# julien-michot/tinyopt

Measured on AMD Instinct MI355X. Metric: LM iterations/s (batched dense n<=50), higher is better.
Workload: dtype f32

## Files before the change

### include/tinyopt_amd.h

```cpp
#ifndef TINYOPT_AMD_H_
#define TINYOPT_AMD_H_

#include <stddef.h>
#include <stdint.h>

#ifdef __cplusplus
extern "C" {
#endif

#define TOA_VERSION 1

#define TOA_OK 0
#define TOA_E_ARG (-1)
#define TOA_E_HIP (-2)
#define TOA_E_NOMEM (-3)
#define TOA_E_UNSUPPORTED (-4)
#define TOA_E_RCCL (-5)

#define TOA_F32 0
#define TOA_F64 1

#define TOA_MODEL_DENSE_ROW 1
#define TOA_MODEL_GAUSSIAN_PRIOR 2
#define TOA_MODEL_SQRT2 3
// ... 206 lines not shown
#define TOA_DIFF_NUM_CENTRAL 2
#define TOA_DIFF_NUM_FAST_CENTRAL 3
typedef struct toa_jit_spec {
  int32_t dtype, num_params, residuals_per_item, scalars_per_item, header_scalars;
  int32_t manifold;
  int32_t kind;
  int32_t x_scalars;
  const char* plus_body;
  int32_t diff;
  float diff_h;
  union {
    int32_t reserved[4];
    int32_t large_n;
    struct {
      int32_t toa_pad0_;
      int32_t shared_scalars;
    };
  };
} toa_jit_spec;
int toa_model_compile_ex(toa_handle h, const toa_jit_spec* spec, const char* body, toa_jit_model* out, char* log_out, size_t log_cap);
int toa_jit_set_cache_dir(const char* dir);
int toa_jit_model_info(toa_jit_model m, int* from_cache, int* xdim);
int toa_jit_model_stats(toa_jit_model m, int* wg_per_cu, int* lds_bytes_per_wg, int* num_regs, int* scratch_bytes);
int toa_model_destroy(toa_jit_model m);
int toa_jit_lm_run(toa_handle h, toa_jit_model model, int num_items, int64_t P, const void* data_dev, void* x_dev,
                   const toa_options* options, const toa_results* results, uint64_t* counters_dev);
int toa_jit_accumulate(toa_handle h, toa_jit_model model, int num_items, int64_t P, const void* data_dev, const void* x_dev,
                       int want_grad, void* g_dev, void* H_dev, double* cost_dev, int32_t* nres_dev);
int toa_jit_check_gradient(toa_handle h, toa_jit_model model, int num_items, int64_t P, const void* data_dev, const void* x_dev,
                           double eps, int method, int check_H, double* max_dist_dev, int32_t* ok_dev);
int toa_jit_eval(toa_handle h, toa_jit_model model, int num_items, int64_t P, const void* data_dev, const void* x_dev, void* res_dev,
                 void* J_dev);
typedef struct toa_gd_options {
  float lr;
  int32_t reserved[7];
} toa_gd_options;
void toa_gd_options_default(toa_gd_options* o);
int toa_jit_gd_run(toa_handle h, toa_jit_model model, int num_items, int64_t P, const void* data_dev, void* x_dev,
                   const toa_options* options, const toa_gd_options* gd, const toa_results* results, uint64_t* counters_dev);
int toa_jit_lm_run_split(toa_handle h, toa_jit_model model, int num_items, int64_t P, const void* data_dev, void* x_dev,
                         const toa_options* options, const toa_results* results, uint64_t* counters_dev, int splits);
int toa_jit_lm_begin(toa_handle h, toa_jit_model model, int num_items, int64_t P, const void* data_dev, void* x_dev,
                     const toa_options* options, const toa_results* results, void* state_dev);
int toa_jit_lm_step(toa_handle h, toa_jit_model model, int num_items, int64_t P, const void* data_dev, void* x_dev,
                    const toa_options* options, const toa_results* results, uint64_t* counters_dev, void* state_dev,
                    int32_t* active_dev);
// ... 77 lines not shown
```

### include/tinyopt_amd/tinyopt.hpp

```cpp
#pragma once

#include <array>
#include <chrono>
#include <cstdint>
#include <functional>
#include <iostream>
#include <limits>
#include <stdexcept>
#include <string>
#include <algorithm>
#include <type_traits>
#include <utility>
#include <vector>

#include "../tinyopt_amd.h"

namespace tinyopt_amd {

enum StopReason : int {
  kOutOfMemory = -4, kSolverFailed = -3, kSystemHasNaNOrInf = -2, kSkipped = -1, kNone = 0, kMinError, kMinRelError,
  kMinDeltaNorm, kMinGradNorm, kMaxIters, kMaxNoDecr, kMaxConsecNoDecr, kTimedOut, kUserStopped
};

struct Options {
// ... 348 lines not shown
    if (kind_ == TOA_JIT_COST_GGN_MULTI) detail::refuse_cost_ggn_multi("no ragged batches (bind_ragged)");
    if (kS_ > 0) detail::refuse_shared("no ragged batches (bind_ragged)");
    return RaggedJitModel<Scalar>(*this, counts, data, header);
  }
  const std::string& compile_log() const { return log_; }
  toa_jit_model handle() const { return h_; }
  const Context& ctx() const { return *ctx_; }
  int n() const { return n_; }
  int residuals_per_item() const { return kR_; }
  int item_scalars() const { return kD_; }
  int header_scalars() const { return kH_; }
  int xdim() const { return xdim_; }
  int diff() const { return diff_; }
  int manifold() const { return manifold_; }
  int kind() const { return kind_; }
  bool large_n() const { return large_n_; }
  int shared_scalars() const { return kS_; }
  struct PriorBuildStats { int wg_per_cu = 0, num_regs = 0, scratch_bytes = 0; };
  PriorBuildStats stats_prior(bool ragged = false) const {
    PriorBuildStats s;
    check(toa_jit_model_stats_prior(ctx_->get(), h_, ragged ? 1 : 0, &s.wg_per_cu, &s.num_regs, &s.scratch_bytes));
    return s;
  }
  struct BuildStats { int wg_per_cu = 0, lds_bytes_per_wg = 0, num_regs = 0, scratch_bytes = 0; };
  BuildStats stats() const {
    BuildStats s;
    check(toa_jit_model_stats(h_, &s.wg_per_cu, &s.lds_bytes_per_wg, &s.num_regs, &s.scratch_bytes));
    return s;
  }

 private:
  const Context* ctx_;
  toa_jit_model h_ = nullptr;
  int n_, kR_, kD_, kH_, xdim_, diff_, manifold_, kind_;
  bool large_n_;
  int kS_;
  std::string log_;
};
template <typename Scalar>
class PriorTag {
 public:
  bool has_prior() const { return prior_rows_ >= 0; }
  toa_prior prior_pod() const {
    toa_prior p{};
    p.mu_dev = prior_mu_.data(); p.W_dev = prior_W_.data(); p.rows = prior_rows_;
    return p;
  }

 protected:
  void set_prior(const JitResidual<Scalar>& res, int64_t P, const Scalar* mu, const Scalar* W, int rows) {
// ... 892 lines not shown
```

### tinyopt_amd/_capi.py

```python
from __future__ import annotations

import ctypes as C
import os

_HERE = os.path.dirname(os.path.abspath(__file__))
LIB_PATH = os.environ.get("TINYOPT_AMD_LIB", os.path.join(_HERE, "libtinyopt_amd.so"))

F32, F64 = 0, 1
MODEL_DENSE_ROW, MODEL_GAUSSIAN_PRIOR, MODEL_SQRT2, MODEL_SE3_REPROJ, MODEL_CIRCLE_FIT, MODEL_DENSE_ROW_AD6 = 1, 2, 3, 4, 5, 6
MODEL_TESTFN = 7
MODEL_MAHA_PRIOR = 8
MODEL_SE3_PRIOR = 9
MODEL_DENSE_ROW_NATURAL = 10
MODEL_DENSE_ROW_AD = 11

STOP_NAMES = {
    -4: "kOutOfMemory", -3: "kSolverFailed", -2: "kSystemHasNaNOrInf", -1: "kSkipped", 0: "kNone",
    1: "kMinError", 2: "kMinRelError", 3: "kMinDeltaNorm", 4: "kMinGradNorm", 5: "kMaxIters",
    6: "kMaxNoDecr", 7: "kMaxConsecNoDecr", 8: "kTimedOut", 9: "kUserStopped",
}


class ToaOptions(C.Structure):
    _fields_ = [
# ... 107 lines not shown
    "toa_dense_row_synth": (C.c_int, [_P, C.c_int, C.c_int, C.c_int, C.c_int64, C.c_uint64, C.c_int64, _P, _P, _P]),
    "toa_accumulate": (C.c_int, [_P, C.c_int, C.c_int, C.c_int, C.c_int, C.c_int64, _P, _P, C.c_int, _P, _P, _P, _P]),
    "toa_solve_damped": (C.c_int, [_P, C.c_int, C.c_int, C.c_int64, _P, _P, C.c_double, _P, _P]),
    "toa_inv_cov": (C.c_int, [_P, C.c_int, C.c_int, C.c_int64, _P, _P, _P]),
    "toa_lm_run": (C.c_int, [_P, C.c_int, C.c_int, C.c_int, C.c_int, C.c_int64, _P, _P, C.POINTER(ToaOptions),
                             C.POINTER(ToaResults), _P]),
    "toa_ba_lists_run": (C.c_int, [_P, C.c_int, C.c_int, C.c_int, C.c_int, C.c_int64, _P, _P, _P, _P, _P, C.POINTER(ToaOptions),
                                   C.POINTER(ToaResults), _P, C.c_double]),
    "toa_ba_run_constant": (C.c_int, [_P, C.c_int, C.c_int, C.c_int, C.c_int64, _P, _P, C.POINTER(ToaOptions), C.POINTER(ToaResults), _P,
                                      C.POINTER(ToaBaConstant)]),
    "toa_ba_lists_run_constant": (C.c_int, [_P, C.c_int, C.c_int, C.c_int, C.c_int, C.c_int64, _P, _P, _P, _P, _P, C.POINTER(ToaOptions),
                                            C.POINTER(ToaResults), _P, C.c_double, C.POINTER(ToaBaConstant)]),
    "toa_model_compile": (C.c_int, [_P, C.c_int, C.c_int, C.c_int, C.c_int, C.c_int, C.c_char_p, C.POINTER(_P), C.c_char_p, C.c_size_t]),
    "toa_abi_version": (C.c_int, []),
    "toa_device_count": (C.c_int, [C.POINTER(C.c_int)]),
    "toa_set_tuning": (C.c_int, [_P, C.POINTER(ToaTuning)]),
    "toa_get_tuning": (C.c_int, [_P, C.POINTER(ToaTuning)]),
    "toa_debug_timeline": (C.c_int, [_P, C.c_char_p]),
    "toa_model_compile_ex": (C.c_int, [_P, C.POINTER(ToaJitSpec), C.c_char_p, C.POINTER(_P), C.c_char_p, C.c_size_t]),
    "toa_jit_set_cache_dir": (C.c_int, [C.c_char_p]),
    "toa_lm_step_log": (C.c_int, [_P, C.c_int, C.c_int, C.c_int64, _P, _P, _P, _P]),
    "toa_jit_model_info": (C.c_int, [_P, C.POINTER(C.c_int), C.POINTER(C.c_int)]),
    "toa_jit_model_stats": (C.c_int, [_P, C.POINTER(C.c_int), C.POINTER(C.c_int), C.POINTER(C.c_int), C.POINTER(C.c_int)]),
    "toa_model_destroy": (C.c_int, [_P]),
    "toa_jit_lm_run": (C.c_int, [_P, _P, C.c_int, C.c_int64, _P, _P, C.POINTER(ToaOptions), C.POINTER(ToaResults), _P]),
    "toa_jit_accumulate": (C.c_int, [_P, _P, C.c_int, C.c_int64, _P, _P, C.c_int, _P, _P, _P, _P]),
    "toa_jit_check_gradient": (C.c_int, [_P, _P, C.c_int, C.c_int64, _P, _P, C.c_double, C.c_int, C.c_int, _P, _P]),
    "toa_jit_eval": (C.c_int, [_P, _P, C.c_int, C.c_int64, _P, _P, _P, _P]),
    "toa_jit_lm_run_ragged": (C.c_int, [_P, _P, _P, _P, C.c_int, C.c_int64, C.c_int64, _P, _P, C.POINTER(ToaOptions), C.POINTER(ToaResults), _P,
                                        C.c_uint32]),
    "toa_jit_gd_run_ragged": (C.c_int, [_P, _P, _P, _P, C.c_int, C.c_int64, C.c_int64, _P, _P, C.POINTER(ToaOptions), C.POINTER(ToaGdOptions),
                                        C.POINTER(ToaResults), _P, C.c_uint32]),
    "toa_jit_accumulate_ragged": (C.c_int, [_P, _P, _P, _P, C.c_int, C.c_int64, C.c_int64, _P, _P, C.c_int, _P, _P, _P, _P]),
    "toa_jit_eval_ragged": (C.c_int, [_P, _P, _P, _P, C.c_int, C.c_int64, C.c_int64, _P, _P, _P, _P]),
    "toa_jit_model_stats_ragged": (C.c_int, [_P, _P, C.POINTER(C.c_int), C.POINTER(C.c_int), C.POINTER(C.c_int)]),
    "toa_jit_lm_run_prior": (C.c_int, [_P, _P, C.c_int, C.c_int64, _P, _P, C.POINTER(ToaPrior), C.POINTER(ToaOptions), C.POINTER(ToaResults), _P]),
    "toa_jit_accumulate_prior": (C.c_int, [_P, _P, C.c_int, C.c_int64, _P, _P, C.POINTER(ToaPrior), C.c_int, _P, _P, _P, _P]),
    "toa_jit_lm_run_ragged_prior": (C.c_int, [_P, _P, _P, _P, C.c_int, C.c_int64, C.c_int64, _P, _P, C.POINTER(ToaPrior), C.POINTER(ToaOptions),
                                              C.POINTER(ToaResults), _P, C.c_uint32]),
    "toa_jit_accumulate_ragged_prior": (C.c_int, [_P, _P, _P, _P, C.c_int, C.c_int64, C.c_int64, _P, _P, C.POINTER(ToaPrior), C.c_int, _P, _P, _P, _P]),
    "toa_jit_model_stats_prior": (C.c_int, [_P, _P, C.c_int, C.POINTER(C.c_int), C.POINTER(C.c_int), C.POINTER(C.c_int)]),
    "toa_jit_lm_run_bounds": (C.c_int, [_P, _P, C.c_int, C.c_int64, _P, _P, C.POINTER(ToaBounds), C.POINTER(ToaPrior), C.POINTER(ToaOptions),
                                        C.POINTER(ToaResults), _P]),
    "toa_jit_lm_run_ragged_bounds": (C.c_int, [_P, _P, _P, _P, C.c_int, C.c_int64, C.c_int64, _P, _P, C.POINTER(ToaBounds), C.POINTER(ToaPrior),
                                               C.POINTER(ToaOptions), C.POINTER(ToaResults), _P, C.c_uint32]),
    "toa_jit_accumulate_bounds": (C.c_int, [_P, _P, C.c_int, C.c_int64, _P, _P, C.POINTER(ToaBounds), C.POINTER(ToaPrior), C.c_int, _P, _P, _P, _P]),
# ... 54 lines not shown
```

### tinyopt_amd/api.py

```python
from __future__ import annotations

import contextlib
import copy
import ctypes as C
import enum
import functools
import time

import numpy as np
from dataclasses import dataclass, field
from typing import Optional

import torch

from . import _capi
from ._capi import (F32, F64, MODEL_DENSE_ROW_AD, MODEL_DENSE_ROW_NATURAL, MODEL_TESTFN, MODEL_MAHA_PRIOR, MODEL_SE3_PRIOR, MODEL_CIRCLE_FIT, MODEL_DENSE_ROW, MODEL_DENSE_ROW_AD6, MODEL_GAUSSIAN_PRIOR, MODEL_SE3_REPROJ,
                    MODEL_SQRT2, ToaBaConstant, ToaBounds, ToaGdOptions, ToaJitSpec, ToaLbfgsOptions, ToaOptions, ToaPrior, ToaResults, ToaShared, check)


class StopReason(enum.IntEnum):
    kOutOfMemory = -4
    kSolverFailed = -3
    kSystemHasNaNOrInf = -2
    kSkipped = -1
# ... 797 lines not shown
        self._h = C.c_void_p()
        log = C.create_string_buffer(1 << 16)
        spec = ToaJitSpec()
        spec.dtype, spec.num_params, spec.residuals_per_item = _dtype_code(dtype), self.n, self.kR
        spec.scalars_per_item, spec.header_scalars = self.kD, self.kH
        spec.manifold, spec.kind = self.MANIFOLDS[manifold], self.KINDS[kind]
        spec.diff, spec.diff_h = self.DIFFS[diff], self.diff_h
        spec.large_n = 1 if self.large_n else 0
        spec.shared_scalars = self.kS
        if manifold == "user":
            if not plus_body or int(x_scalars) < 1:
                raise ValueError('manifold="user" needs plus_body (the body of x (+) d) and x_scalars')
            spec.x_scalars, spec.plus_body = int(x_scalars), plus_body.encode()
        rc = self.ctx.lib.toa_model_compile_ex(self.ctx.h, C.byref(spec), body.encode(), C.byref(self._h), log, len(log))
        self.compile_log = log.value.decode(errors="replace")
        check(rc)
        fc = C.c_int(0)
        check(self.ctx.lib.toa_jit_model_info(self._h, C.byref(fc), None))
        self.from_cache = bool(fc.value)

    def stats(self) -> dict:
        v = [C.c_int(0) for _ in range(4)]
        check(self.ctx.lib.toa_jit_model_stats(self._h, *[C.byref(t) for t in v]))
        return dict(wg_per_cu=v[0].value, lds_bytes_per_wg=v[1].value, num_regs=v[2].value, scratch_bytes=v[3].value)

    @staticmethod
    def set_cache_dir(path: Optional[str], ctx: Optional["Context"] = None) -> None:
        check((ctx or default_context()).lib.toa_jit_set_cache_dir(None if path is None else path.encode()))

    def bind(self, data: Optional[torch.Tensor], header: Optional[torch.Tensor] = None, items: int = 1,
             shared: Optional[torch.Tensor] = None) -> "JitModel":
        kS = getattr(self, "kS", 0)
        if shared is None:
            if kS:
                raise ValueError(f"bind: a model with shared_scalars = {kS} needs shared=, the batch's [items, {kS}] table")
            return JitModel(self, data, header, items)
        if not kS:
            raise ValueError("bind: shared= is the table of a model with shared_scalars > 0; this model has none")
        m = JitModel(self, data, header, items)
        if not isinstance(shared, torch.Tensor) or tuple(shared.shape) != (m.items, kS):
            raise ValueError(f"bind: shared must be an [items, shared_scalars] = [{m.items}, {kS}] tensor, not "
                             f"{list(shared.shape) if isinstance(shared, torch.Tensor) else type(shared).__name__}")
        if shared.dtype != self.dtype or shared.device != m.packed.device:
            raise ValueError(f"bind: shared must have the model's dtype {self.dtype} on the data's device {m.packed.device}, not {shared.dtype} on {shared.device}")
        m.shared = shared.contiguous()
        return m

# ... 728 lines not shown
```

### tinyopt_amd/csrc/jet.hpp

```cpp
#pragma once
#include <hip/hip_runtime.h>

#include <cmath>

namespace toa {

using ::sqrt; using ::sin; using ::cos; using ::tan; using ::atan; using ::atan2; using ::tanh;
using ::exp; using ::log; using ::pow; using ::fabs; using std::abs;
using ::isnan; using ::isinf; using ::isfinite; using ::signbit;
using ::acos; using ::asin; using ::sinh; using ::cosh; using ::cbrt; using ::exp2; using ::log2; using ::log10;
using ::log1p; using ::expm1; using ::hypot; using ::erf; using ::erfc; using ::floor; using ::ceil; using ::fmax;
using ::fmin; using ::fdim; using ::fma; using ::copysign;

template <typename T, int N>
struct Jet {
  T a;
  T v[N];

  __host__ __device__ Jet() : a(T(0)) {
#pragma unroll
    for (int i = 0; i < N; ++i) v[i] = T(0);
  }
  __host__ __device__ Jet(T value) : a(value) {
#pragma unroll
    for (int i = 0; i < N; ++i) v[i] = T(0);
  }
  __host__ __device__ Jet(T value, int k) : a(value) {
#pragma unroll
    for (int i = 0; i < N; ++i) v[i] = (i == k) ? T(1) : T(0);
  }
  __host__ __device__ Jet& operator+=(const Jet& y) { *this = *this + y; return *this; }
  __host__ __device__ Jet& operator-=(const Jet& y) { *this = *this - y; return *this; }
  __host__ __device__ Jet& operator*=(const Jet& y) { *this = *this * y; return *this; }
  __host__ __device__ Jet& operator/=(const Jet& y) { *this = *this / y; return *this; }
  __host__ __device__ Jet& operator+=(T s) { a += s; return *this; }
  __host__ __device__ Jet& operator-=(T s) { a -= s; return *this; }
  __host__ __device__ Jet& operator*=(T s) { *this = *this * s; return *this; }
  __host__ __device__ Jet& operator/=(T s) { *this = *this / s; return *this; }
};

#define TOA_JET_FN template <typename T, int N> __host__ __device__ inline
#define TOA_JET_LOOP _Pragma("unroll") for (int i = 0; i < N; ++i)

TOA_JET_FN Jet<T, N> operator+(const Jet<T, N>& f) { return f; }
TOA_JET_FN Jet<T, N> operator-(const Jet<T, N>& f) { Jet<T, N> r; r.a = -f.a; TOA_JET_LOOP r.v[i] = -f.v[i]; return r; }
TOA_JET_FN Jet<T, N> operator+(const Jet<T, N>& f, const Jet<T, N>& g) {
  Jet<T, N> r; r.a = f.a + g.a; TOA_JET_LOOP r.v[i] = f.v[i] + g.v[i]; return r;
}
TOA_JET_FN Jet<T, N> operator+(const Jet<T, N>& f, T s) { Jet<T, N> r = f; r.a += s; return r; }
TOA_JET_FN Jet<T, N> operator+(T s, const Jet<T, N>& f) { Jet<T, N> r = f; r.a += s; return r; }
TOA_JET_FN Jet<T, N> operator-(const Jet<T, N>& f, const Jet<T, N>& g) {
  Jet<T, N> r; r.a = f.a - g.a; TOA_JET_LOOP r.v[i] = f.v[i] - g.v[i]; return r;
}
TOA_JET_FN Jet<T, N> operator-(const Jet<T, N>& f, T s) { Jet<T, N> r = f; r.a -= s; return r; }
TOA_JET_FN Jet<T, N> operator-(T s, const Jet<T, N>& f) { Jet<T, N> r = -f; r.a += s; return r; }
TOA_JET_FN Jet<T, N> operator*(const Jet<T, N>& f, const Jet<T, N>& g) {
  Jet<T, N> r; r.a = f.a * g.a; TOA_JET_LOOP r.v[i] = f.a * g.v[i] + f.v[i] * g.a; return r;
}
TOA_JET_FN Jet<T, N> operator*(const Jet<T, N>& f, T s) { Jet<T, N> r; r.a = f.a * s; TOA_JET_LOOP r.v[i] = f.v[i] * s; return r; }
TOA_JET_FN Jet<T, N> operator*(T s, const Jet<T, N>& f) { return f * s; }
TOA_JET_FN Jet<T, N> operator/(const Jet<T, N>& f, const Jet<T, N>& g) {
// ... 162 lines not shown
TOA_JET_FN bool isnan(const Jet<T, N>& f) { return f.a != f.a; }
TOA_JET_FN bool isnormal(const Jet<T, N>& f) {
  const T m = f.a < T(0) ? -f.a : f.a;
  return ::isfinite(f.a) && m >= (sizeof(T) == 4 ? T(1.17549435e-38f) : T(2.2250738585072014e-308));
}
TOA_JET_FN bool signbit(const Jet<T, N>& f) { return ::signbit(f.a); }
TOA_JET_FN int fpclassify(const Jet<T, N>& f) {
  if (f.a != f.a) return 0;
  if (::isinf(f.a)) return 1;
  if (f.a == T(0)) return 2;
  return isnormal(f) ? 4 : 3;
}
TOA_JET_FN bool isless(const Jet<T, N>& f, const Jet<T, N>& g) { return f.a < g.a; }
TOA_JET_FN bool isgreater(const Jet<T, N>& f, const Jet<T, N>& g) { return f.a > g.a; }
TOA_JET_FN bool islessequal(const Jet<T, N>& f, const Jet<T, N>& g) { return f.a <= g.a; }
TOA_JET_FN bool isgreaterequal(const Jet<T, N>& f, const Jet<T, N>& g) { return f.a >= g.a; }
TOA_JET_FN bool islessgreater(const Jet<T, N>& f, const Jet<T, N>& g) { return f.a < g.a || f.a > g.a; }
TOA_JET_FN bool isunordered(const Jet<T, N>& f, const Jet<T, N>& g) { return f.a != f.a || g.a != g.a; }
TOA_JET_FN bool IsFinite(const Jet<T, N>& f) { return isfinite(f); }
TOA_JET_FN bool IsNaN(const Jet<T, N>& f) { return isnan(f); }
TOA_JET_FN bool IsNormal(const Jet<T, N>& f) { return isnormal(f); }
TOA_JET_FN bool IsInfinite(const Jet<T, N>& f) { return isinf(f); }

#undef TOA_JET_FN
#undef TOA_JET_LOOP

}
```

### tinyopt_amd/csrc/jit.hip

```cpp
#include <dlfcn.h>
#include <glob.h>
#include <sys/stat.h>
#include <unistd.h>

#include <cstdint>
#include <mutex>
#include <string>
#include <vector>

#include "kernels.hpp"
#include "gd_kernels.hpp"
#include "lbfgs_kernels.hpp"
#include "large_model_geom.hpp"
#include "_obj/jit_embed.inc"

struct JitObject {
  hipModule_t module = nullptr;
  hipFunction_t fn[5] = {};
  bool from_cache = false;
  int wg_per_cu = 0;
  int regs = 0, scratch = 0;
};
enum { kFnFused = 0, kFnSeam = 1 };
enum { kFnWideInit = 0, kFnWidePart, kFnWideStep, kFnWideStop, kFnWidePers };
// ... 7 lines not shown
  std::string prefix;
};
struct JitEvalGeom {
  size_t lds_j = 0, lds = 0;
  int items_j = 0, items = 0;
};
struct toa_jit_model_s {
  bool large_n = false;
  toa::LargeModelRows mr = {};
  enum { kObjWide = 2 * kForms, kObjEval = kObjWide + 1, kObjLarge = kObjEval + 2, kObjLbfgs = kObjLarge + 1, kObjects = kObjLbfgs + 2 };
  JitObject obj[kObjects];
  JitObject& form(int form, int robust) { return obj[2 * form + robust]; }
  JitObject& wide() { return obj[kObjWide]; }
  JitObject& eval(bool ragged) { return obj[kObjEval + (ragged ? 1 : 0)]; }
  JitObject& large() { return obj[kObjLarge]; }
  JitObject& lbfgs(bool ragged) { return obj[kObjLbfgs + (ragged ? 1 : 0)]; }
  JitGeom geom[2];
  JitEvalGeom ev_geom[2];
  int lbfgs_wg[2][17] = {};
  std::mutex build_mu;
  int dtype = 0, kN = 0, kR = 0, kD = 0, kH = 0, device = 0;
  int manifold = 0, kind = 0, xdim = 0, x_scalars = 0;
  int kS = 0;
  bool row_model = false;
  size_t memo_bytes = 0;
  hipStream_t last_stream = nullptr;
  std::vector<hipStream_t> streams;
  void used_on(hipStream_t s) {
    last_stream = s;
    for (hipStream_t t : streams) if (t == s) return;
    streams.push_back(s);
  }
  std::string functor_src, model_expr, arch;
  std::string wide_model_expr;
  bool wide_row_model = false;
  int diff = 0;
  double diff_h = 0;
  toa_jit_spec spec = {};
  std::string body;
  int body_kind = 0;
  bool seam_only = false;
  struct Twin { int method; double h; toa_jit_model_s* m; };
  std::vector<Twin> twins;
};

namespace {
// ... 270 lines not shown
  return ((dtype == TOA_F32 ? toa::WaveLds<float>::bytes(n) : toa::WaveLds<double>::bytes(n)) + 15) & ~size_t(15);
}

struct RowGeom { size_t stage_bytes, lds_wave, lds_wg; int carve_off; };
static RowGeom row_stage_geometry(toa_jit_model m, int waves_override) {
  const int n = m->kN, sz = m->dtype == TOA_F32 ? 4 : 8;
  const bool ad = m->kind != TOA_JIT_ACCUMULATE;
  int table = 0;
  if (ad && m->manifold == TOA_MANIFOLD_SE3) table = (12 * 7 * sz + 15) & ~15;
  if (ad && m->manifold == TOA_MANIFOLD_USER) {
    const int cwmax = jit_flag_int("TOA_AD_CW", 12);
    const int chunks = (n + cwmax - 1) / cwmax, cw = (n + chunks - 1) / chunks;
    table = (chunks * m->x_scalars * (cw + 1) * sz + 15) & ~15;
  }
  const int waves = waves_override ? waves_override : jit_flag_int("TOA_ROW_WAVES", TOA_ROW_WAVES);
  RowGeom g;
  g.stage_bytes = size_t(toa::RowStageGeom::make(sz, n, m->kR, m->kD, ad || jit_flag_int("TOA_ROW_SINGLE", TOA_ROW_SINGLE),
                                                 jit_flag_int("TOA_ROW_NBUF", TOA_ROW_NBUF), waves, table, m->kS).bytes);
  const size_t dead = std::min(m->dtype == TOA_F32 ? toa::WaveLds<float>::pass_dead_bytes(n) : toa::WaveLds<double>::pass_dead_bytes(n), g.stage_bytes);
  g.carve_off = int(g.stage_bytes - dead);
  g.lds_wave = carve_bytes(m->dtype, n) + size_t(g.carve_off);
  g.lds_wg = 4 * g.lds_wave;
  return g;
}

static bool is_cost_model(toa_jit_model m) { return m->kind == TOA_JIT_COST || m->kind == TOA_JIT_COST_GRAD; }
static bool is_hess_model(toa_jit_model m) { return m->kind == TOA_JIT_COST_HESS; }
static int refuse_hess_model(const std::string& who, const std::string& what) {
  return toa_fail(TOA_E_UNSUPPORTED, who + ": a second-order scalar cost (TOA_JIT_COST_HESS) runs in the uniform one-launch form through toa_jit_lm_run "
                                           "(LM / GN), toa_jit_accumulate, toa_jit_check_gradient and toa_jit_model_stats only: " + what);
}
static bool is_ggn_model(toa_jit_model m) { return m->kind == TOA_JIT_COST_GGN; }
static int refuse_ggn_model(const std::string& who, const std::string& what) {
  return toa_fail(TOA_E_UNSUPPORTED, who + ": a rank-one second-order scalar cost (TOA_JIT_COST_GGN) runs in the uniform one-launch form through toa_jit_lm_run "
                                           "(LM / GN), toa_jit_accumulate, toa_jit_check_gradient and toa_jit_model_stats only: " + what);
}
static bool is_ggn_multi_model(toa_jit_model m) { return m->kind == TOA_JIT_COST_GGN_MULTI; }
static int refuse_ggn_multi_model(const std::string& who, const std::string& what) {
  return toa_fail(TOA_E_UNSUPPORTED, who + ": a multi-output second-order scalar cost (TOA_JIT_COST_GGN_MULTI) runs in the uniform one-launch form through "
                                           "toa_jit_lm_run (LM / GN), toa_jit_accumulate, their _prior and _shared forms, toa_jit_check_gradient and "
                                           "toa_jit_model_stats only: " + what);
}
static bool is_item_cost_model(toa_jit_model m) { return is_ggn_model(m) || is_ggn_multi_model(m); }

static bool is_shared_model(toa_jit_model m) { return m->kS > 0; }
static int refuse_shared_model(const std::string& who, const std::string& what) {
// ... 529 lines not shown
            ", 0, TOA_ROBUST_>";
  } else if (row_model) {
    const std::string f = std::string("toa::UserFunctor<") + tname + ">";
    const std::string mf = std::to_string(spec->manifold);
    model = std::string("toa::RowModel<") + tname + ", " + std::to_string(lay.nbm) + ", " + std::to_string(lay.thin) + ", " +
            (spec->kind == TOA_JIT_ACCUMULATE ? f : std::string("toa::AdRowFunctor<") + tname + ", " + f + ", " + mf + ">") + ", " + mf + ", TOA_ROBUST_>";
  } else {
    model = std::string("toa::JetModel<") + tname + ", toa::UserFunctor<" + tname + ">, " + std::to_string(spec->manifold) + ", TOA_ROBUST_>";
  }
  const std::string jet_model = std::string("toa::JetModel<") + tname + ", toa::UserFunctor<" + tname + ">, " + std::to_string(spec->manifold) + ">";
  toa_jit_model_s* m = new (std::nothrow) toa_jit_model_s;
  if (!m) return toa_fail(TOA_E_NOMEM, "out of host memory");
  m->dtype = dtype; m->kN = n; m->kR = kR; m->kD = kD; m->kH = kH;
  m->manifold = spec->manifold; m->kind = spec->kind; m->row_model = row_model;
  m->x_scalars = user_manifold ? spec->x_scalars : 0;
  m->xdim = spec->manifold == TOA_MANIFOLD_SE3 ? 12 : (user_manifold ? spec->x_scalars : n);
  m->device = h->device;
  m->functor_src = src; m->model_expr = model; m->arch = arch;
  m->wide_row_model = row_model && n > 12 && kS == 0;
  m->kS = kS;
  m->diff = diff; m->diff_h = numeric ? diff_h : 0.0;
  m->spec = *spec; m->spec.plus_body = nullptr;
  m->body = body; m->body_kind = body_kind; m->seam_only = seam_only;
  if (large) {
    m->large_n = true;
    m->row_model = false; m->wide_row_model = false;
    if (int rc = build_large_model(m, log_out, log_cap)) { delete m; return rc; }
    *out = m;
    return TOA_OK;
  }
  if (cost_kind) {
    if (int rc = build_cost_variant(m, log_out, log_cap)) { delete m; return rc; }
    *out = m;
    return TOA_OK;
  }
  if (hess_kind) {
    if (int rc = build_hess_variant(m, log_out, log_cap)) { delete m; return rc; }
    *out = m;
    return TOA_OK;
  }
  if (ggn_kind || ggn_multi_kind) {
    m->wide_row_model = false;
    if (int rc = build_ggn_variant(m, log_out, log_cap)) { delete m; return rc; }
    *out = m;
    return TOA_OK;
  }
  {
    std::string wm = model;
    wm.replace(wm.find("TOA_ROBUST_"), 11, "true");
    m->wide_model_expr = m->wide_row_model ? wm : jet_model;
  }
  if (int rc = build_variant(m, 0, log_out, log_cap)) { delete m; return rc; }
  *out = m;
  return TOA_OK;
}
extern "C" {

int toa_model_compile_ex(toa_handle h, const toa_jit_spec* spec, const char* body, toa_jit_model* out, char* log_out, size_t log_cap) {
  if (!spec) return toa_fail(TOA_E_ARG, "toa_model_compile: null argument");
  return compile_model(h, spec, body, spec->kind, double(spec->diff_h), false, out, log_out, log_cap);
}

int toa_model_compile(toa_handle h, int dtype, int num_params, int residuals_per_item, int scalars_per_item, int header_scalars,
                      const char* residual_body, toa_jit_model* out, char* log_out, size_t log_cap) {
  toa_jit_spec spec;
  std::memset(&spec, 0, sizeof(spec));
  spec.dtype = dtype; spec.num_params = num_params; spec.residuals_per_item = residuals_per_item;
  spec.scalars_per_item = scalars_per_item; spec.header_scalars = header_scalars;
  return toa_model_compile_ex(h, &spec, residual_body, out, log_out, log_cap);
}

int toa_jit_model_info(toa_jit_model m, int* from_cache, int* xdim) {
  if (!m) return toa_fail(TOA_E_ARG, "toa_jit_model_info: null model");
  if (from_cache) *from_cache = (m->large_n ? m->large() : m->form(0, 0)).from_cache ? 1 : 0;
  if (xdim) *xdim = m->xdim;
  return TOA_OK;
}

int toa_jit_model_stats(toa_jit_model m, int* wg_per_cu, int* lds_bytes_per_wg, int* num_regs, int* scratch_bytes) {
  if (!m) return toa_fail(TOA_E_ARG, "toa_jit_model_stats: null model");
  TOA_ON_DEVICE(m->device);
  if (m->large_n) {
    const hipFunction_t fn = m->mr.rows_j;
    int v = 0;
    if (wg_per_cu) { if (hipModuleOccupancyMaxActiveBlocksPerMultiprocessor(&v, fn, 256, m->mr.lds_j) != hipSuccess || v < 1) v = 1; *wg_per_cu = v; }
    if (lds_bytes_per_wg) *lds_bytes_per_wg = int(m->mr.lds_j);
    if (num_regs) { HIP_TRY(hipFuncGetAttribute(&v, HIP_FUNC_ATTRIBUTE_NUM_REGS, fn)); *num_regs = v; }
    if (scratch_bytes) { HIP_TRY(hipFuncGetAttribute(&v, HIP_FUNC_ATTRIBUTE_LOCAL_SIZE_BYTES, fn)); *scratch_bytes = v; }
    return TOA_OK;
  }
  const JitObject& V = m->form(0, 0);
  if (wg_per_cu) *wg_per_cu = V.wg_per_cu;
  if (lds_bytes_per_wg) *lds_bytes_per_wg = int(m->geom[0].lds_wg);
  int v = 0;
  if (num_regs) { HIP_TRY(hipFuncGetAttribute(&v, HIP_FUNC_ATTRIBUTE_NUM_REGS, V.fn[kFnFused])); *num_regs = v; }
  if (scratch_bytes) { HIP_TRY(hipFuncGetAttribute(&v, HIP_FUNC_ATTRIBUTE_LOCAL_SIZE_BYTES, V.fn[kFnFused])); *scratch_bytes = v; }
  return TOA_OK;
}

int toa_model_destroy(toa_jit_model m) {
  if (!m) return TOA_OK;
  TOA_ON_DEVICE(m->device);
  for (hipStream_t s : m->streams) {
    if (stream_is_capturing(s))
      return toa_fail(TOA_E_UNSUPPORTED, "toa_model_destroy: a stream this model was launched on is being captured; end the capture first "
                                         "(and keep the model for as long as a graph that recorded its kernels may be launched)");
    (void)hipGetLastError();
  }
  for (hipStream_t s : m->streams) {
    if (hipStreamSynchronize(s) != hipSuccess) (void)hipGetLastError();
  }
  for (const toa_jit_model_s::Twin& t : m->twins) (void)toa_model_destroy(t.m);
  for (JitObject& O : m->obj) if (O.module) (void)hipModuleUnload(O.module);
  delete m;
  return TOA_OK;
}

}

// ... 830 lines not shown
  size_t gbytes = 0;
  if (hipError_t e = hipModuleGetGlobal(&gp, &gbytes, mod, "toa_eval_geom"); e != hipSuccess || gbytes != sizeof(geom))
    return fail("the code object does not carry its LDS geometry", e);
  if (hipError_t e = hipMemcpyDtoH(geom, gp, sizeof(geom)); e != hipSuccess) return fail("reading the LDS geometry", e);
  if (geom[0] < 16 || geom[2] < 16 || geom[1] < 1 || geom[3] < 1 || size_t(geom[0]) * 4 > 160 * 1024 || size_t(geom[2]) * 4 > 160 * 1024)
    return fail("implausible LDS geometry", hipErrorInvalidValue);
  for (int k = 0; k < 2; ++k)
    if (size_t(geom[2 * k]) * 4 > 64 * 1024)
      if (hipError_t e = hipFuncSetAttribute(reinterpret_cast<const void*>(fn[k]), hipFuncAttributeMaxDynamicSharedMemorySize, geom[2 * k] * 4); e != hipSuccess)
        return fail("raising the dynamic LDS limit to " + std::to_string(geom[2 * k] * 4) + " bytes per workgroup", e);
  JitObject& E = m->eval(ragged);
  JitEvalGeom& G = m->ev_geom[ragged ? 1 : 0];
  E.fn[kFnRowsJ] = fn[0]; E.fn[kFnRows] = fn[1];
  G.lds_j = size_t(geom[0]); G.lds = size_t(geom[2]);
  G.items_j = geom[1]; G.items = geom[3];
  E.from_cache = cached;
  E.module = mod;
  return TOA_OK;
}
static int ensure_eval(toa_jit_model m, hipStream_t stream, const bool ragged) {
  return lazy_build(m, stream, [&] { return m->eval(ragged).module != nullptr; },
                    "run-time model: the Eval kernels of this model are compiled on their first use (toa_jit_eval), which cannot "
                    "happen while the stream is being captured; run the call once before hipStreamBeginCapture",
                    [&] { return build_eval(m, ragged); });
}

static int launch_eval(const char* who, toa_handle h, toa_jit_model model, int num_items, int64_t P, const void* data_dev, const void* x_dev, void* res_dev,
                       void* J_dev, const toa::RaggedArgs* rag) {
  if (int rc = ensure_eval(model, h->stream, rag != nullptr)) return rc;
  const JitEvalGeom& E = model->ev_geom[rag ? 1 : 0];
  model->used_on(h->stream);
  const bool want_j = J_dev != nullptr;
  const hipFunction_t fn = model->eval(rag != nullptr).fn[want_j ? kFnRowsJ : kFnRows];
  const size_t pw = want_j ? E.lds_j : E.lds;
  const long long it = want_j ? E.items_j : E.items;
  const long long nss = ((long long)num_items + it - 1) / it;
  const long long want_units = (long long)h->num_cus * 32 * 4;
  long long spu = nss;
  if ((long long)P < want_units) spu = std::max(1ll, std::min(nss, nss * (long long)P / want_units));
  const long long upp = (nss + spu - 1) / spu;
  const long long grid = std::max(1ll, std::min(((long long)P * upp + 3) / 4, (long long)h->num_cus * 16));
  const void* d = data_dev;
  const void* x = x_dev;
  long long Pll = P;
  int items = num_items, spui = int(spu);
  toa::RaggedArgs ra = rag ? *rag : toa::RaggedArgs();
  void* args[] = {&d, &x, &Pll, &items, &res_dev, &J_dev, &spui, &ra};
// ... 168 lines not shown
```

### tinyopt_amd/csrc/row_model.hpp

```cpp
#pragma once
#include "shared.hpp"
#include "row_stage_geom.hpp"
#ifndef TOA_ROW_SINGLE
#define TOA_ROW_SINGLE 1
#endif
#ifndef TOA_ROW_XREGS
#define TOA_ROW_XREGS 0
#endif
#ifndef TOA_ROW_ABL
#define TOA_ROW_ABL 0
#endif

namespace toa {

__device__ __forceinline__ float seed_one(bool b, float) {
  return __builtin_bit_cast(float, __builtin_amdgcn_readfirstlane(b ? 0x3f800000 : 0));
}
__device__ __forceinline__ double seed_one(bool b, double) {
  const unsigned hi = unsigned(__builtin_amdgcn_readfirstlane(b ? 0x3ff00000 : 0));
  return __builtin_bit_cast(double, (unsigned long long)hi << 32);
}
template <typename T, int CW>
struct ChunkSeededX {
  const T* xs;
  int c0;
  __device__ __forceinline__ Jet<T, CW> operator[](int j) const {
    Jet<T, CW> r;
    r.a = xs[j];
#pragma unroll
    for (int s = 0; s < CW; ++s) r.v[s] = seed_one(j == c0 + s, T(0));
    return r;
  }
};
template <typename T, int CW>
struct ChunkSeededD {
  int c0;
  __device__ __forceinline__ Jet<T, CW> operator[](int a) const {
    Jet<T, CW> r;
    r.a = T(0);
#pragma unroll
    for (int s = 0; s < CW; ++s) r.v[s] = (a == c0 + s) ? T(1) : T(0);
    return r;
  }
};
template <typename T, typename F, int MANIFOLD = 0>
struct AdRowFunctor {
  static constexpr int kN = F::kN, kR = F::kR, kD = F::kD, kH = F::kH;
  static_assert(MANIFOLD != 1 || F::kN == 6, "TOA_MANIFOLD_SE3: one pose, six tangent dimensions");
  static constexpr int kX = MANIFOLD == 1 ? 12 : (MANIFOLD == 2 ? FunctorX<F>::value : F::kN);
  template <class S, class XA_, class DA_, class XP_>
  static __device__ __forceinline__ void plus(const XA_& x, const DA_& d, XP_&& xp) { F::template plus<S>(x, d, xp); }
  static constexpr bool kManual = true;
  static constexpr bool kComputeBound = true;
  static constexpr bool kIndexedOperands = true;
#ifndef TOA_AD_CW
// ... 506 lines not shown
```

Measured before the change: 13.26 million.

## Add lazy seed proxies for forward-mode AD to skip dense seed vectors

Chunk-seeded inputs now return a lightweight SeedVar/SeedTerm proxy instead of a full Jet with a one-hot derivative vector. Addition, subtraction and scalar scaling of these proxies touch only the single seeded lane, using a wave-uniform branch. Any other operation first expands the proxy to a dense Jet. The aim is to cut per-element derivative arithmetic and register pressure in user residual bodies. If a user body fails to compile with the proxy types, the build retries with dense seeds, and a stats query reports which path is in use.

```diff
diff --git a/include/tinyopt_amd.h b/include/tinyopt_amd.h
--- a/include/tinyopt_amd.h
+++ b/include/tinyopt_amd.h
@@ -252,6 +252,7 @@
 int toa_jit_set_cache_dir(const char* dir);
 int toa_jit_model_info(toa_jit_model m, int* from_cache, int* xdim);
 int toa_jit_model_stats(toa_jit_model m, int* wg_per_cu, int* lds_bytes_per_wg, int* num_regs, int* scratch_bytes);
+int toa_jit_model_ad_seeds(toa_jit_model m, int* lazy_seeds);
 int toa_model_destroy(toa_jit_model m);
 int toa_jit_lm_run(toa_handle h, toa_jit_model model, int num_items, int64_t P, const void* data_dev, void* x_dev,
                    const toa_options* options, const toa_results* results, uint64_t* counters_dev);
diff --git a/include/tinyopt_amd/tinyopt.hpp b/include/tinyopt_amd/tinyopt.hpp
--- a/include/tinyopt_amd/tinyopt.hpp
+++ b/include/tinyopt_amd/tinyopt.hpp
@@ -394,10 +394,11 @@
     check(toa_jit_model_stats_prior(ctx_->get(), h_, ragged ? 1 : 0, &s.wg_per_cu, &s.num_regs, &s.scratch_bytes));
     return s;
   }
-  struct BuildStats { int wg_per_cu = 0, lds_bytes_per_wg = 0, num_regs = 0, scratch_bytes = 0; };
+  struct BuildStats { int wg_per_cu = 0, lds_bytes_per_wg = 0, num_regs = 0, scratch_bytes = 0, ad_lazy_seeds = -1; };
   BuildStats stats() const {
     BuildStats s;
     check(toa_jit_model_stats(h_, &s.wg_per_cu, &s.lds_bytes_per_wg, &s.num_regs, &s.scratch_bytes));
+    check(toa_jit_model_ad_seeds(h_, &s.ad_lazy_seeds));
     return s;
   }
 
diff --git a/tinyopt_amd/_capi.py b/tinyopt_amd/_capi.py
--- a/tinyopt_amd/_capi.py
+++ b/tinyopt_amd/_capi.py
@@ -153,6 +153,7 @@
     "toa_lm_step_log": (C.c_int, [_P, C.c_int, C.c_int, C.c_int64, _P, _P, _P, _P]),
     "toa_jit_model_info": (C.c_int, [_P, C.POINTER(C.c_int), C.POINTER(C.c_int)]),
     "toa_jit_model_stats": (C.c_int, [_P, C.POINTER(C.c_int), C.POINTER(C.c_int), C.POINTER(C.c_int), C.POINTER(C.c_int)]),
+    "toa_jit_model_ad_seeds": (C.c_int, [_P, C.POINTER(C.c_int)]),
     "toa_model_destroy": (C.c_int, [_P]),
     "toa_jit_lm_run": (C.c_int, [_P, _P, C.c_int, C.c_int64, _P, _P, C.POINTER(ToaOptions), C.POINTER(ToaResults), _P]),
     "toa_jit_accumulate": (C.c_int, [_P, _P, C.c_int, C.c_int64, _P, _P, C.c_int, _P, _P, _P, _P]),
diff --git a/tinyopt_amd/api.py b/tinyopt_amd/api.py
--- a/tinyopt_amd/api.py
+++ b/tinyopt_amd/api.py
@@ -843,7 +843,10 @@
     def stats(self) -> dict:
         v = [C.c_int(0) for _ in range(4)]
         check(self.ctx.lib.toa_jit_model_stats(self._h, *[C.byref(t) for t in v]))
-        return dict(wg_per_cu=v[0].value, lds_bytes_per_wg=v[1].value, num_regs=v[2].value, scratch_bytes=v[3].value)
+        lazy = C.c_int(-1)
+        check(self.ctx.lib.toa_jit_model_ad_seeds(self._h, C.byref(lazy)))
+        return dict(wg_per_cu=v[0].value, lds_bytes_per_wg=v[1].value, num_regs=v[2].value, scratch_bytes=v[3].value,
+                    ad_lazy_seeds=lazy.value)
 
     @staticmethod
     def set_cache_dir(path: Optional[str], ctx: Optional["Context"] = None) -> None:
diff --git a/tinyopt_amd/csrc/jet.hpp b/tinyopt_amd/csrc/jet.hpp
--- a/tinyopt_amd/csrc/jet.hpp
+++ b/tinyopt_amd/csrc/jet.hpp
@@ -1,7 +1,21 @@
 #pragma once
+#if defined(__HIPCC__) || defined(__HIPCC_RTC__)
 #include <hip/hip_runtime.h>
+#else
+#define __host__
+#define __device__
+#define __forceinline__ inline
+#endif
 
 #include <cmath>
+#include <type_traits>
+#if !(defined(__HIPCC__) || defined(__HIPCC_RTC__))
+using std::isnan; using std::isinf; using std::isfinite; using std::signbit;
+#endif
+
+#ifndef TOA_AD_LAZY_SEEDS
+#define TOA_AD_LAZY_SEEDS 1
+#endif
 
 namespace toa {
 
@@ -11,6 +25,9 @@
 using ::acos; using ::asin; using ::sinh; using ::cosh; using ::cbrt; using ::exp2; using ::log2; using ::log10;
 using ::log1p; using ::expm1; using ::hypot; using ::erf; using ::erfc; using ::floor; using ::ceil; using ::fmax;
 using ::fmin; using ::fdim; using ::fma; using ::copysign;
+
+template <typename T, int N> struct SeedVar;
+template <typename T, int N> struct SeedTerm;
 
 template <typename T, int N>
 struct Jet {
@@ -37,6 +54,10 @@
   __host__ __device__ Jet& operator-=(T s) { a -= s; return *this; }
   __host__ __device__ Jet& operator*=(T s) { *this = *this * s; return *this; }
   __host__ __device__ Jet& operator/=(T s) { *this = *this / s; return *this; }
+  __host__ __device__ Jet& operator+=(const SeedTerm<T, N>& y) { *this = *this + y; return *this; }
+  __host__ __device__ Jet& operator-=(const SeedTerm<T, N>& y) { *this = *this - y; return *this; }
+  __host__ __device__ Jet& operator+=(const SeedVar<T, N>& y) { *this = *this + y; return *this; }
+  __host__ __device__ Jet& operator-=(const SeedVar<T, N>& y) { *this = *this - y; return *this; }
 };
 
 #define TOA_JET_FN template <typename T, int N> __host__ __device__ inline
@@ -245,6 +266,141 @@
 TOA_JET_FN bool IsNormal(const Jet<T, N>& f) { return isnormal(f); }
 TOA_JET_FN bool IsInfinite(const Jet<T, N>& f) { return isinf(f); }
 
+__host__ __device__ __forceinline__ float seed_one(bool b, float) {
+#if defined(__HIP_DEVICE_COMPILE__)
+  return __builtin_bit_cast(float, __builtin_amdgcn_readfirstlane(b ? 0x3f800000 : 0));
+#else
+  return b ? 1.0f : 0.0f;
+#endif
+}
+__host__ __device__ __forceinline__ double seed_one(bool b, double) {
+#if defined(__HIP_DEVICE_COMPILE__)
+  const unsigned hi = unsigned(__builtin_amdgcn_readfirstlane(b ? 0x3ff00000 : 0));
+  return __builtin_bit_cast(double, (unsigned long long)hi << 32);
+#else
+  return b ? 1.0 : 0.0;
+#endif
+}
+template <int N>
+__host__ __device__ __forceinline__ bool seed_in_chunk(int k) {
+#if defined(__HIP_DEVICE_COMPILE__)
+  k = __builtin_amdgcn_readfirstlane(k);
+#endif
+  return unsigned(k) < unsigned(N);
+}
+template <typename T, int N>
+struct SeedVar {
+  T a;
+  int k;
+  __host__ __device__ operator Jet<T, N>() const {
+    Jet<T, N> r; r.a = a; TOA_JET_LOOP r.v[i] = seed_one(k == i, T(0)); return r;
+  }
+};
+template <typename T, int N>
+struct SeedTerm {
+  T a, s;
+  int k;
+  __host__ __device__ operator Jet<T, N>() const {
+    Jet<T, N> r; r.a = a; TOA_JET_LOOP r.v[i] = seed_one(k == i, T(0)) * s; return r;
+  }
+};
+TOA_JET_FN SeedTerm<T, N> operator*(const SeedVar<T, N>& x, T s) { return SeedTerm<T, N>{x.a * s, s, x.k}; }
+TOA_JET_FN SeedTerm<T, N> operator*(T s, const SeedVar<T, N>& x) { return SeedTerm<T, N>{x.a * s, s, x.k}; }
+TOA_JET_FN SeedTerm<T, N> operator-(const SeedVar<T, N>& x) { return SeedTerm<T, N>{-x.a, T(-1), x.k}; }
+TOA_JET_FN SeedTerm<T, N> operator-(const SeedTerm<T, N>& x) { return SeedTerm<T, N>{-x.a, -x.s, x.k}; }
+TOA_JET_FN SeedVar<T, N> operator+(const SeedVar<T, N>& x) { return x; }
+TOA_JET_FN SeedTerm<T, N> operator+(const SeedTerm<T, N>& x) { return x; }
+TOA_JET_FN SeedVar<T, N> operator+(const SeedVar<T, N>& x, T s) { return SeedVar<T, N>{x.a + s, x.k}; }
+TOA_JET_FN SeedVar<T, N> operator+(T s, const SeedVar<T, N>& x) { return SeedVar<T, N>{x.a + s, x.k}; }
+TOA_JET_FN SeedVar<T, N> operator-(const SeedVar<T, N>& x, T s) { return SeedVar<T, N>{x.a - s, x.k}; }
+TOA_JET_FN Jet<T, N> operator+(const Jet<T, N>& f, const SeedTerm<T, N>& g) {
+  Jet<T, N> r; r.a = f.a + g.a;
+  if (seed_in_chunk<N>(g.k)) { TOA_JET_LOOP r.v[i] = f.v[i] + seed_one(g.k == i, T(0)) * g.s; }
+  else { TOA_JET_LOOP r.v[i] = f.v[i]; }
+  return r;
+}
+TOA_JET_FN Jet<T, N> operator+(const SeedTerm<T, N>& g, const Jet<T, N>& f) {
+  Jet<T, N> r; r.a = g.a + f.a;
+  if (seed_in_chunk<N>(g.k)) { TOA_JET_LOOP r.v[i] = seed_one(g.k == i, T(0)) * g.s + f.v[i]; }
+  else { TOA_JET_LOOP r.v[i] = f.v[i]; }
+  return r;
+}
+TOA_JET_FN Jet<T, N> operator-(const Jet<T, N>& f, const SeedTerm<T, N>& g) {
+  Jet<T, N> r; r.a = f.a - g.a;
+  if (seed_in_chunk<N>(g.k)) { TOA_JET_LOOP r.v[i] = f.v[i] - seed_one(g.k == i, T(0)) * g.s; }
+  else { TOA_JET_LOOP r.v[i] = f.v[i]; }
+  return r;
+}
+TOA_JET_FN Jet<T, N> operator-(const SeedTerm<T, N>& g, const Jet<T, N>& f) {
+  Jet<T, N> r; r.a = g.a - f.a;
+  if (seed_in_chunk<N>(g.k)) { TOA_JET_LOOP r.v[i] = seed_one(g.k == i, T(0)) * g.s - f.v[i]; }
+  else { TOA_JET_LOOP r.v[i] = -f.v[i]; }
+  return r;
+}
+TOA_JET_FN Jet<T, N> operator+(const Jet<T, N>& f, const SeedVar<T, N>& g) {
+  Jet<T, N> r; r.a = f.a + g.a;
+  if (seed_in_chunk<N>(g.k)) { TOA_JET_LOOP r.v[i] = f.v[i] + seed_one(g.k == i, T(0)); }
+  else { TOA_JET_LOOP r.v[i] = f.v[i]; }
+  return r;
+}
+TOA_JET_FN Jet<T, N> operator+(const SeedVar<T, N>& g, const Jet<T, N>& f) {
+  Jet<T, N> r; r.a = g.a + f.a;
+  if (seed_in_chunk<N>(g.k)) { TOA_JET_LOOP r.v[i] = seed_one(g.k == i, T(0)) + f.v[i]; }
+  else { TOA_JET_LOOP r.v[i] = f.v[i]; }
+  return r;
+}
+TOA_JET_FN Jet<T, N> operator-(const Jet<T, N>& f, const SeedVar<T, N>& g) {
+  Jet<T, N> r; r.a = f.a - g.a;
+  if (seed_in_chunk<N>(g.k)) { TOA_JET_LOOP r.v[i] = f.v[i] - seed_one(g.k == i, T(0)); }
+  else { TOA_JET_LOOP r.v[i] = f.v[i]; }
+  return r;
+}
+TOA_JET_FN Jet<T, N> operator-(const SeedVar<T, N>& g, const Jet<T, N>& f) {
+  Jet<T, N> r; r.a = g.a - f.a;
+  if (seed_in_chunk<N>(g.k)) { TOA_JET_LOOP r.v[i] = seed_one(g.k == i, T(0)) - f.v[i]; }
+  else { TOA_JET_LOOP r.v[i] = -f.v[i]; }
+  return r;
+}
+template <class X> struct SeedProxy { static constexpr bool value = false; using Dense = const X&; };
+template <typename T, int N> struct SeedProxy<SeedVar<T, N>> { static constexpr bool value = true; using Dense = Jet<T, N>; };
+template <typename T, int N> struct SeedProxy<SeedTerm<T, N>> { static constexpr bool value = true; using Dense = Jet<T, N>; };
+template <class X> __host__ __device__ __forceinline__ typename SeedProxy<X>::Dense seed_dense(const X& x) { return x; }
+#define TOA_SEED_BINARY(fn)                                                                                              \
+  template <class A, class B, std::enable_if_t<SeedProxy<A>::value || SeedProxy<B>::value, int> = 0>                     \
+  __host__ __device__ inline auto fn(const A& a, const B& b) -> decltype(fn(seed_dense(a), seed_dense(b))) {             \
+    return fn(seed_dense(a), seed_dense(b));                                                                             \
+  }
+#define TOA_SEED_UNARY(fn)                                                                                               \
+  template <class A, std::enable_if_t<SeedProxy<A>::value, int> = 0>                                                     \
+  __host__ __device__ inline auto fn(const A& a) -> decltype(fn(seed_dense(a))) {                                        \
+    return fn(seed_dense(a));                                                                                            \
+  }
+#define TOA_SEED_TERNARY(fn)                                                                                             \
+  template <class A, class B, class C,                                                                                   \
+            std::enable_if_t<SeedProxy<A>::value || SeedProxy<B>::value || SeedProxy<C>::value, int> = 0>                \
+  __host__ __device__ inline auto fn(const A& a, const B& b, const C& c)                                                 \
+      -> decltype(fn(seed_dense(a), seed_dense(b), seed_dense(c))) {                                                     \
+    return fn(seed_dense(a), seed_dense(b), seed_dense(c));                                                              \
+  }
+TOA_SEED_BINARY(operator+) TOA_SEED_BINARY(operator-) TOA_SEED_BINARY(operator*) TOA_SEED_BINARY(operator/)
+TOA_SEED_BINARY(operator<) TOA_SEED_BINARY(operator>) TOA_SEED_BINARY(operator<=) TOA_SEED_BINARY(operator>=)
+TOA_SEED_BINARY(operator==) TOA_SEED_BINARY(operator!=)
+TOA_SEED_UNARY(abs) TOA_SEED_UNARY(log) TOA_SEED_UNARY(exp) TOA_SEED_UNARY(sqrt) TOA_SEED_UNARY(cos) TOA_SEED_UNARY(sin)
+TOA_SEED_UNARY(tan) TOA_SEED_UNARY(atan) TOA_SEED_UNARY(tanh) TOA_SEED_UNARY(log10) TOA_SEED_UNARY(log1p) TOA_SEED_UNARY(expm1)
+TOA_SEED_UNARY(acos) TOA_SEED_UNARY(asin) TOA_SEED_UNARY(sinh) TOA_SEED_UNARY(cosh) TOA_SEED_UNARY(floor) TOA_SEED_UNARY(ceil)
+TOA_SEED_UNARY(cbrt) TOA_SEED_UNARY(exp2) TOA_SEED_UNARY(log2) TOA_SEED_UNARY(erf) TOA_SEED_UNARY(erfc) TOA_SEED_UNARY(norm)
+TOA_SEED_UNARY(BesselJ0) TOA_SEED_UNARY(BesselJ1) TOA_SEED_UNARY(isfinite) TOA_SEED_UNARY(isinf) TOA_SEED_UNARY(isnan)
+TOA_SEED_UNARY(isnormal) TOA_SEED_UNARY(signbit) TOA_SEED_UNARY(fpclassify) TOA_SEED_UNARY(IsFinite) TOA_SEED_UNARY(IsNaN)
+TOA_SEED_UNARY(IsNormal) TOA_SEED_UNARY(IsInfinite)
+TOA_SEED_BINARY(atan2) TOA_SEED_BINARY(pow) TOA_SEED_BINARY(copysign) TOA_SEED_BINARY(hypot) TOA_SEED_BINARY(fmax)
+TOA_SEED_BINARY(fmin) TOA_SEED_BINARY(fdim) TOA_SEED_BINARY(BesselJn) TOA_SEED_BINARY(cyl_bessel_j) TOA_SEED_BINARY(midpoint)
+TOA_SEED_BINARY(isless) TOA_SEED_BINARY(isgreater) TOA_SEED_BINARY(islessequal) TOA_SEED_BINARY(isgreaterequal)
+TOA_SEED_BINARY(islessgreater) TOA_SEED_BINARY(isunordered)
+TOA_SEED_TERNARY(hypot) TOA_SEED_TERNARY(fma) TOA_SEED_TERNARY(lerp)
+#undef TOA_SEED_BINARY
+#undef TOA_SEED_UNARY
+#undef TOA_SEED_TERNARY
+
 #undef TOA_JET_FN
 #undef TOA_JET_LOOP
 
diff --git a/tinyopt_amd/csrc/jit.hip b/tinyopt_amd/csrc/jit.hip
--- a/tinyopt_amd/csrc/jit.hip
+++ b/tinyopt_amd/csrc/jit.hip
@@ -53,6 +53,7 @@
   int dtype = 0, kN = 0, kR = 0, kD = 0, kH = 0, device = 0;
   int manifold = 0, kind = 0, xdim = 0, x_scalars = 0;
   int kS = 0;
+  int ad_seeds = -1;
   bool row_model = false;
   size_t memo_bytes = 0;
   hipStream_t last_stream = nullptr;
@@ -369,6 +370,13 @@
   g.lds_wave = carve_bytes(m->dtype, n) + size_t(g.carve_off);
   g.lds_wg = 4 * g.lds_wave;
   return g;
+}
+
+static bool ad_dense_fallback(toa_jit_model m, int rc) {
+  if (rc != TOA_E_ARG || m->ad_seeds != 1) return false;
+  m->functor_src = "#undef TOA_AD_LAZY_SEEDS\n#define TOA_AD_LAZY_SEEDS 0\n" + m->functor_src;
+  m->ad_seeds = 0;
+  return true;
 }
 
 static bool is_cost_model(toa_jit_model m) { return m->kind == TOA_JIT_COST || m->kind == TOA_JIT_COST_GRAD; }
@@ -944,10 +952,14 @@
   m->diff = diff; m->diff_h = numeric ? diff_h : 0.0;
   m->spec = *spec; m->spec.plus_body = nullptr;
   m->body = body; m->body_kind = body_kind; m->seam_only = seam_only;
+  if (spec->kind == TOA_JIT_RESIDUAL && body_kind == TOA_JIT_RESIDUAL && !numeric && spec->manifold == TOA_MANIFOLD_EUCLID)
+    m->ad_seeds = jit_flag_int("TOA_AD_LAZY_SEEDS", 1) != 0 ? 1 : 0;
   if (large) {
     m->large_n = true;
     m->row_model = false; m->wide_row_model = false;
-    if (int rc = build_large_model(m, log_out, log_cap)) { delete m; return rc; }
+    int rc = build_large_model(m, log_out, log_cap);
+    if (ad_dense_fallback(m, rc)) rc = build_large_model(m, log_out, log_cap);
+    if (rc) { delete m; return rc; }
     *out = m;
     return TOA_OK;
   }
@@ -972,7 +984,9 @@
     wm.replace(wm.find("TOA_ROBUST_"), 11, "true");
     m->wide_model_expr = m->wide_row_model ? wm : jet_model;
   }
-  if (int rc = build_variant(m, 0, log_out, log_cap)) { delete m; return rc; }
+  int rc = build_variant(m, 0, log_out, log_cap);
+  if (ad_dense_fallback(m, rc)) rc = build_variant(m, 0, log_out, log_cap);
+  if (rc) { delete m; return rc; }
   *out = m;
   return TOA_OK;
 }
@@ -1017,6 +1031,12 @@
   int v = 0;
   if (num_regs) { HIP_TRY(hipFuncGetAttribute(&v, HIP_FUNC_ATTRIBUTE_NUM_REGS, V.fn[kFnFused])); *num_regs = v; }
   if (scratch_bytes) { HIP_TRY(hipFuncGetAttribute(&v, HIP_FUNC_ATTRIBUTE_LOCAL_SIZE_BYTES, V.fn[kFnFused])); *scratch_bytes = v; }
+  return TOA_OK;
+}
+
+int toa_jit_model_ad_seeds(toa_jit_model m, int* lazy_seeds) {
+  if (!m || !lazy_seeds) return toa_fail(TOA_E_ARG, "toa_jit_model_ad_seeds: null argument");
+  *lazy_seeds = m->ad_seeds;
   return TOA_OK;
 }
 
@@ -1893,7 +1913,11 @@
   return lazy_build(m, stream, [&] { return m->eval(ragged).module != nullptr; },
                     "run-time model: the Eval kernels of this model are compiled on their first use (toa_jit_eval), which cannot "
                     "happen while the stream is being captured; run the call once before hipStreamBeginCapture",
-                    [&] { return build_eval(m, ragged); });
+                    [&] {
+                      int rc = build_eval(m, ragged);
+                      if (!m->row_model && !m->large_n && ad_dense_fallback(m, rc)) rc = build_eval(m, ragged);
+                      return rc;
+                    });
 }
 
 static int launch_eval(const char* who, toa_handle h, toa_jit_model model, int num_items, int64_t P, const void* data_dev, const void* x_dev, void* res_dev,
diff --git a/tinyopt_amd/csrc/row_model.hpp b/tinyopt_amd/csrc/row_model.hpp
--- a/tinyopt_amd/csrc/row_model.hpp
+++ b/tinyopt_amd/csrc/row_model.hpp
@@ -13,24 +13,15 @@
 
 namespace toa {
 
-__device__ __forceinline__ float seed_one(bool b, float) {
-  return __builtin_bit_cast(float, __builtin_amdgcn_readfirstlane(b ? 0x3f800000 : 0));
-}
-__device__ __forceinline__ double seed_one(bool b, double) {
-  const unsigned hi = unsigned(__builtin_amdgcn_readfirstlane(b ? 0x3ff00000 : 0));
-  return __builtin_bit_cast(double, (unsigned long long)hi << 32);
-}
 template <typename T, int CW>
 struct ChunkSeededX {
   const T* xs;
   int c0;
-  __device__ __forceinline__ Jet<T, CW> operator[](int j) const {
-    Jet<T, CW> r;
-    r.a = xs[j];
-#pragma unroll
-    for (int s = 0; s < CW; ++s) r.v[s] = seed_one(j == c0 + s, T(0));
-    return r;
-  }
+#if TOA_AD_LAZY_SEEDS
+  __device__ __forceinline__ SeedVar<T, CW> operator[](int j) const { return SeedVar<T, CW>{xs[j], j - c0}; }
+#else
+  __device__ __forceinline__ Jet<T, CW> operator[](int j) const { return SeedVar<T, CW>{xs[j], j - c0}; }
+#endif
 };
 template <typename T, int CW>
 struct ChunkSeededD {
```

Result: no change. 13.26 million (-0.0%).
